# facebookresearch/seamless_communication

Hardware: AMD Instinct MI355X
Metric: S2ST utterances/sec (and real-time factor), seamlessM4T_v2_large, 10 s audio (higher is better)
Workload: dtype f32 activations x f16 weights, f32 accumulate

## Files before the change

include/seamless_hip_internal.h:

```cpp
#ifndef SEAMLESS_HIP_INTERNAL_H_
#define SEAMLESS_HIP_INTERNAL_H_

#include "seamless_hip.h"

#ifdef __cplusplus
extern "C" {
#endif

int sc_decoder_step_family(sc_model* m, int rows, int caller);

int sc_op_knob(const char* name, int dflt);

int sc_op_force_general_gemm(int on);
int32_t sc_op_voc_pack_plan(const int32_t* h_need, int32_t n, int64_t budget_rows, int32_t* h_group_first, int32_t cap);
int32_t sc_op_voc_tile_first(const int32_t* h_off, int32_t n, int32_t mul, int32_t tile_rows, int32_t* h_first);
int32_t sc_op_last_vocoder_packed_groups(sc_model* m);
int sc_op_single_plane(int on);
int sc_op_layernorm(const float* d_x, const float* d_gamma, const float* d_beta, float* d_y, int32_t rows, int32_t C,
                    int32_t act);
int sc_op_linear(const float* d_x, const void* d_w_f16, const float* d_bias, const float* d_res, float* d_y,
                 int32_t M, int32_t N, int32_t K, int32_t act, float alpha, int32_t split, int32_t force_gemv);
int sc_op_skinny_linear(const float* d_x, const void* d_w_f16, const float* d_bias, const float* d_res, float* d_y,
                        int32_t M, int32_t N, int32_t K, int32_t act, float alpha);
int sc_op_skinny_res_ln(const float* d_in, const void* d_w_f16, const float* d_bias, float* d_x_inout,
// ... 13 lines not shown
int sc_op_dstep_attention(const float* d_proj, int32_t S, const float* d_bias, float* d_kcache, float* d_vcache, int32_t cap,
                          int32_t pos, const int32_t* d_lens, int32_t cross, int32_t nb, int32_t heads, float* d_out);
int sc_op_dstep3_gemv(int32_t mode, const float* d_x, const void* d_w_f16, const float* d_bias, const float* d_gamma,
                      const float* d_beta, const float* d_res, float* d_y, float* d_h, int32_t M, int32_t N, int32_t K, int32_t act,
                      int32_t rg, int32_t shape);
int sc_op_dstep3_argmax(const float* d_x, const void* d_w_f16, int32_t M, int32_t N, int32_t K, int32_t step,
                        int32_t min_step_for_eos, int32_t force_eos_step, int32_t pad_idx, int32_t eos_idx, int32_t unk_idx,
                        float unk_penalty, int32_t* d_idx, float* d_lprob);
int sc_op_chain_bench(int32_t kind, int32_t rows, int32_t n, int32_t reps, float* us_per_kernel);
int sc_op_conv1d(const float* d_x, const void* d_w_f16_packed, const float* d_bias, const float* d_res, float* d_y,
                 int32_t nb, int32_t t_in, int32_t cin, int32_t cout, int32_t k, int32_t stride, int32_t pad,
                 int32_t dil, const int32_t* d_in_lens, int32_t in_act, int32_t act);
int sc_op_pack_conv_weight(const void* d_w_f16, void* d_dst_f16, int32_t cout, int32_t cin, int32_t k);
int sc_op_conv_transpose1d(const float* d_x, const void* d_v_f16, const void* d_g_f16, const float* d_bias,
                           float* d_y, int32_t nb, int32_t t_in, int32_t cin, int32_t cout, int32_t k,
                           int32_t stride, int32_t pad, int32_t in_act);
int sc_op_linear_presplit(const float* d_x, const void* d_w_f16, const float* d_bias, const float* d_res, float* d_y,
                          void* d_yh_f16, void* d_yl_f16, int32_t M, int32_t N, int32_t K, int32_t act, float alpha);
int sc_op_linear_presplit_argmax(const float* d_x, const void* d_w_f16, const float* d_bias, int32_t* d_idx, int32_t M, int32_t N,
                                 int32_t K);
int sc_op_conv1d_presplit(const float* d_x, const void* d_w_f16_packed, const float* d_bias, const float* d_res, float* d_y,
                          void* d_yh_f16, void* d_yl_f16, int32_t nb, int32_t t, int32_t cin, int32_t cout, int32_t k, int32_t pad,
                          int32_t dil, const unsigned char* d_row_valid, int32_t act);
int sc_op_resblock_pair_ps(const float* d_x, const void* d_w1_packed, const float* d_b1, const void* d_w2_packed, const float* d_b2,
                           float* d_out, int32_t nb, int32_t T, int32_t C, int32_t k, int32_t dil);
int sc_op_resblock_pair(const float* d_x, const void* d_w1_packed, const float* d_b1, const void* d_w2_packed,
                        const float* d_b2, float* d_out, int32_t nb, int32_t T, int32_t C, int32_t k, int32_t dil,
                        float slope, const float* d_avg_a, const float* d_avg_b);
int sc_op_mrf_fused(const float* d_x, const void* const* d_w1_packed, const float* const* d_b1, const void* const* d_w2_packed,
                    const float* const* d_b2, float* d_out, int32_t nb, int32_t T, int32_t C, const int32_t* k, const int32_t* dil,
                    float slope);
int sc_op_attention(const float* d_q, const float* d_k, const float* d_v, float* d_out, int32_t nb, int32_t heads,
                    int32_t sq, int32_t skv, int64_t ldq, int64_t ldk, int64_t ldv, int64_t ldo,
                    const int32_t* d_kv_lens, int32_t causal, const float* d_rel_k, int32_t rel_left,
                    int32_t rel_right);
int sc_op_attention_ex(const float* d_q, const float* d_k, const float* d_v, float* d_out, int32_t nb, int32_t heads,
                       int32_t sq, int32_t skv, int64_t ldq, int64_t ldk, int64_t ldv, int64_t ldo,
                       const int32_t* d_kv_lens, int32_t causal, const float* d_rel_k, int32_t rel_left,
                       int32_t rel_right, const int32_t* d_row_off, const float* d_rp_table, int64_t rp_ld,
                       const float* d_q_bias_u, const float* d_q_bias_v, void* d_out_hi, void* d_out_lo, int64_t ldoh);
int sc_op_glu_dwconv(const float* d_x, const float* d_w, float* d_y, int32_t nb, int32_t T, int32_t C, int32_t k,
                     const int32_t* d_lens);
int sc_op_glu_dwconv_ln(const float* d_x, const float* d_w, const float* d_gamma, const float* d_beta, int32_t act, void* d_yh_f16,
                        void* d_yl_f16, int32_t nb, int32_t T, int32_t C, int32_t k, const int32_t* d_lens, int32_t fused);
int sc_op_layernorm2(const float* d_x, const float* d_ga, const float* d_ba, const float* d_gb, const float* d_bb, float* d_y,
                     void* d_yh_f16, void* d_yl_f16, int32_t rows, int32_t C, int32_t fused);
// ... 67 lines not shown
```

seamless_communication_amd/_lib.py:

```python
from __future__ import annotations

import ctypes as C
from pathlib import Path
from typing import Optional

import os

_VARIANT = os.environ.get("SC_LIB_VARIANT", "")
LIB_PATH = Path(__file__).resolve().parent / (f"libseamless_hip.{_VARIANT}.so" if _VARIANT else "libseamless_hip.so")

SC_ABI_VERSION = 10
SC_MAX_UPSAMPLES = 8
SC_MAX_RESBLOCK_KERNELS = 4
SC_MAX_RESBLOCK_DILATIONS = 4
SC_F16, SC_F32, SC_I32 = 0, 1, 2


class SeamlessHipError(RuntimeError):
    pass


class sc_tensor_desc(C.Structure):
    _fields_ = [
        ("name", C.c_char_p),
# ... 147 lines not shown
    "sc_op_last_vocoder_packed_groups": (C.c_int32, [_P]),
    "sc_op_single_plane": (C.c_int, [C.c_int]),
    "sc_op_layernorm": (C.c_int, [_P, _P, _P, _P, _i, _i, _i]),
    "sc_op_linear": (C.c_int, [_P, _P, _P, _P, _P, _i, _i, _i, _i, C.c_float, _i, _i]),
    "sc_op_skinny_linear": (C.c_int, [_P, _P, _P, _P, _P, _i, _i, _i, _i, C.c_float]),
    "sc_op_skinny_res_ln": (C.c_int, [_P, _P, _P, _P, _P, _P, _P, _i, _i, _i, _i]),
    "sc_op_skinny_argmax": (C.c_int, [_P, _P, _i, _i, _i, _i, _i, _i, _i, _i, _i, C.c_float, _P, _P]),
    "sc_op_dstep_res_ln": (C.c_int, [_P, _P, _P, _P, _P, _P, _P, _i, _i, _i, _i]),
    "sc_op_dstep_linear_planes": (C.c_int, [_P, _P, _P, _P, _i, _i, _i, _i]),
    "sc_op_dstep_argmax": (C.c_int, [_P, _P, _i, _i, _i, _i, _i, _i, _i, _i, _i, C.c_float, _i, _P, _P]),
    "sc_op_resblock_pair_ps": (C.c_int, [_P, _P, _P, _P, _P, _P, _i, _i, _i, _i, _i]),
    "sc_op_glu_dwconv_ln": (C.c_int, [_P, _P, _P, _P, _i, _P, _P, _i, _i, _i, _i, _P, _i]),
    "sc_op_layernorm2": (C.c_int, [_P, _P, _P, _P, _P, _P, _P, _P, _i, _i, _i]),
    "sc_op_dstep3_gemv": (C.c_int, [_i, _P, _P, _P, _P, _P, _P, _P, _P, _i, _i, _i, _i, _i, _i]),
    "sc_op_dstep3_argmax": (C.c_int, [_P, _P, _i, _i, _i, _i, _i, _i, _i, _i, _i, C.c_float, _P, _P]),
    "sc_op_chain_bench": (C.c_int, [_i, _i, _i, _i, _P]),
    "sc_op_dstep_attention": (C.c_int, [_P, _i, _P, _P, _P, _i, _i, _P, _i, _i, _i, _P]),
    "sc_op_conv1d": (C.c_int, [_P, _P, _P, _P, _P, _i, _i, _i, _i, _i, _i, _i, _i, _P, _i, _i]),
    "sc_op_pack_conv_weight": (C.c_int, [_P, _P, _i, _i, _i]),
    "sc_op_conv_transpose1d": (C.c_int, [_P, _P, _P, _P, _P, _i, _i, _i, _i, _i, _i, _i, _i]),
    "sc_op_linear_presplit": (C.c_int, [_P, _P, _P, _P, _P, _P, _P, _i, _i, _i, _i, C.c_float]),
    "sc_op_linear_presplit_argmax": (C.c_int, [_P, _P, _P, _P, _i, _i, _i]),
    "sc_op_conv1d_presplit": (C.c_int, [_P, _P, _P, _P, _P, _P, _P, _i, _i, _i, _i, _i, _i, _i, _P, _i]),
    "sc_op_mrf_fused": (C.c_int, [_P, _P, _P, _P, _P, _P, _i, _i, _i, _P, _P, C.c_float]),
    "sc_op_resblock_pair": (C.c_int, [_P, _P, _P, _P, _P, _P, _i, _i, _i, _i, _i, C.c_float, _P, _P]),
    "sc_op_attention": (C.c_int, [_P, _P, _P, _P, _i, _i, _i, _i, C.c_int64, C.c_int64, C.c_int64, C.c_int64, _P, _i,
                                  _P, _i, _i]),
    "sc_op_attention_ex": (C.c_int, [_P, _P, _P, _P, _i, _i, _i, _i, C.c_int64, C.c_int64, C.c_int64, C.c_int64, _P, _i,
                                     _P, _i, _i, _P, _P, C.c_int64, _P, _P, _P, _P, C.c_int64]),
    "sc_op_glu_dwconv": (C.c_int, [_P, _P, _P, _i, _i, _i, _i, _P]),
    "sc_op_argmax": (C.c_int, [_P, _i, _i, _P, _P]),
    "sc_op_beam_candidates": (C.c_int, [_P, C.c_int64, _i, _i, _i, _P, _i, _i, _i, _i, _i, _i, C.c_float, _i, _P, _P, _P, _i, _i, _i,
                                        _P, _P, _i]),
    "sc_op_beam_candidates_banned": (C.c_int, [_P, C.c_int64, _i, _i, _i, _P, _i, _i, _i, _i, _i, _i, C.c_float, _i, _P, _P, _P, _i, _i,
                                               _i, _P, _P, _i, _P, _P, _i]),
    "sc_op_beam_select": (C.c_int, [_P, _P, _P, _P, _P, _P, _P, _P, _P, _P, _P, _P, _P, _P, _i, _P, _P, _i, _i, _i, _i, _i, _i, _i, _i,
                                    _i, C.c_float]),
    "sc_op_beam_compact": (C.c_int, [_P, _P, _P, _P, _P, _P, _P, _P, _P, _i, _i, _i, _i, _i, _i]),
    "sc_op_gather_cache": (C.c_int, [_P, _P, _P, _i, _i, _i, _i, _i, C.c_int64]),
    "sc_op_row_token_lprob": (C.c_int, [_P, C.c_int64, _i, _i, _i, _i, _P]),
    "sc_op_dstep_attention_ex": (C.c_int, [_P, _i, _P, _P, _P, _i, _i, _i, _P, _i, _i, _i, _P, _P, _P, _P, _i, _P, _P]),
    "sc_op_engine_step_close": (C.c_int, [_P, _P, _i, _i, _i, _i, _i, _i, _i, C.c_float, _P, _P, _i, _i, _P, _P, _P, _P, _P, _P, _P, _P]),
    "sc_op_engine_admit": (C.c_int, [_P, _i, _i, _i, _i, _P, _P, _P, _P, _P, _P, _P, _P, _P]),
    "sc_op_engine_set_slots": (C.c_int, [_P, _i, _i, _i, _P, _P, _P, _P]),
    "sc_op_engine_retire": (C.c_int, [_P, _P, _P, _i, _i, _i, _i, _P, _P, _P, _P, _P]),
    "sc_op_dstep3_embed_ex": (C.c_int, [_P, _P, C.c_float, _P, _i, _P, _P, _i, _i, _i, _i, _i, _P]),
# ... 96 lines not shown
```

seamless_communication_amd/csrc/api.hip:

```cpp
#include <atomic>
#include <cstring>
#include <map>
#include <mutex>
#include <set>

#include "../../include/seamless_hip_internal.h"
#include "engine.h"
#include "model.h"

using namespace sc;

struct sc_model {
    Model m;
};

struct sc_engine {
    std::unique_ptr<Engine> e;
    int device = 0;
    const void* weights = nullptr;
    std::set<sc_model*> attached;
};

static std::mutex g_attach_mu;
static std::map<Engine*, sc_engine*> g_engine_owner;
// ... 1200 lines not shown
    try {
        launch_split_f32(d_x, hi, lo, (int64_t)n, g_op_stream);
        Model tmp;
        Conv c;
        c.w = static_cast<const __half*>(d_w_f16_packed);
        c.b = d_bias;
        c.cout = cout;
        c.cin = cin;
        c.k = k;
        c.kpad = (int)align_up((int64_t)cin * k, 32);
        conv1d_presplit(tmp, hi, lo, c, d_res, d_y, static_cast<__half*>(d_yh_f16), static_cast<__half*>(d_yl_f16), nb, t, pad, dil,
                        d_row_valid, act);
        SC_HIP(hipStreamSynchronize(g_op_stream));
    } catch (...) {
        (void)hipFree(hi);
        (void)hipFree(lo);
        throw;
    }
    (void)hipFree(hi);
    (void)hipFree(lo);
    SC_API_END
}

int sc_op_resblock_pair_ps(const float* d_x, const void* d_w1_packed, const float* d_b1, const void* d_w2_packed, const float* d_b2,
                           float* d_out, int32_t nb, int32_t T, int32_t C, int32_t k, int32_t dil) {
    SC_API_BEGIN
    SC_CHECK(d_x && d_w1_packed && d_w2_packed && d_out && C % 32 == 0 && (k & 1), "sc_op_resblock_pair_ps: bad argument");
    OpScratch scratch;
    const size_t n = (size_t)nb * T * C;
    const bool one = g_op_single.load() != 0;
    __half* xh = scratch.get<__half>(n);
    __half* xl = one ? nullptr : scratch.get<__half>(n);
    __half* th = scratch.get<__half>(n);
    __half* tl = one ? nullptr : scratch.get<__half>(n);
    launch_lrelu_split_f32(d_x, 0.1f, xh, xl, (int64_t)n, g_op_stream);
    Model tmp;
    Conv c1, c2;
    c1.w = static_cast<const __half*>(d_w1_packed), c1.b = d_b1, c1.cin = c1.cout = C, c1.k = k, c1.kpad = C * k;
    c2.w = static_cast<const __half*>(d_w2_packed), c2.b = d_b2, c2.cin = c2.cout = C, c2.k = k, c2.kpad = C * k;
    conv1d_presplit(tmp, xh, xl, c1, nullptr, nullptr, th, tl, nb, T, (k * dil - dil) / 2, dil, nullptr, ACT_NONE, 0, nullptr, 0.1f, one ? 0 : 1);
    conv1d_presplit(tmp, th, tl, c2, d_x, d_out, nullptr, nullptr, nb, T, (k - 1) / 2, 1, nullptr, ACT_NONE, 0, nullptr, 0.1f, one ? 0 : 1);
    SC_HIP(hipStreamSynchronize(g_op_stream));
    SC_API_END
}

int sc_op_resblock_pair(const float* d_x, const void* d_w1_packed, const float* d_b1, const void* d_w2_packed,
// ... 576 lines not shown
```

seamless_communication_amd/csrc/common.cpp:

```cpp
#include "common.h"
#include <cstdlib>
#include <cstring>

namespace sc {

static thread_local char g_err[1024] = "";

void set_error(const char* fmt, ...) {
    va_list ap;
    va_start(ap, fmt);
    vsnprintf(g_err, sizeof(g_err), fmt, ap);
    va_end(ap);
}

const char* get_error() { return g_err; }

namespace knob {
namespace {
struct Knob {
    const char* name;
    int kind;
    const char* what;
};
const Knob knob_table[] = {
    {"SC_DEBUG_NUMERICS", 0, "honour the switches that change results"},
    {"SC_DEBUG_FILL", 0, "fill fresh scratch blocks with NaN (tests)"},
    {"SC_SPLIT_MODE", 1, "1: Conformer products on the hi fp16 plane only (precision study)"},
    {"SC_DECODER_GEN1", 1, "decoder step on the first-generation kernels"},
    {"SC_DECODER_GEN2", 1, "decoder step on the second-generation chain"},
    {"SC_DECODE_STEPWISE", 1, "teacher-forced pass step by step instead of one batched forward"},
    {"SC_VOC_SPLIT", 1, "vocoder ResBlock products on both fp16 planes of their activations again (bit 0 wide stages, bit 2 narrow stages); default: hi plane only"},
    {"SC_GEMM_GENERAL", 0, "general GEMM kernel instead of the fast path"}, {"SC_GEMM_PF2", 0, "GEMM prefetch depth"},
    {"SC_GEMM_GROUP_M", 0, "GEMM workgroup order"}, {"SC_GEMM_TILE", 0, "GEMM tile override"},
    {"SC_PS_TILE", 0, "DMA GEMM: largest tile"}, {"SC_PS_MIN256", 0, "DMA GEMM: tiles needed for 256 x 256"},
    {"SC_PS_MIN128", 0, "DMA GEMM: tiles needed for 128 x 128"},
    {"SC_PRESPLIT", 0, "0: Conformer operands split on the fly"}, {"SC_ENC_FUSE", 0, "0: separate Conformer element-wise launches"},
    {"SC_D3_RG_SMALL", 0, "decoder step: rows per row group, N = 1024 products"}, {"SC_D3_RG_FFN", 0, "decoder step: rows per row group, FFN-in"},
    {"SC_G3_STATIONARY", 0, "row-group products of wide steps: 0 one workgroup per row group, n = workgroup budget of the weight-stationary launch"},
    {"SC_G3_TILES", 0, "0: FFN-out of wide steps on the weight-stationary row-group walk instead of tile-owning waves"},
    {"SC_G3_TOUCH", 0, "weight-stationary products: bit 0 cooperative L2 touch of the activations, bit 1 K slices per XCD (FFN-out); default 3"},
    {"SC_D3_FFN_IN", 0, "decoder step: FFN-in workgroup shape"}, {"SC_D3_FFN_OUT", 0, "decoder step: FFN-out workgroup shape"},
    {"SC_T2U_GROUPS", 0, "NAR T2U: length buckets"}, {"SC_T2U_PACKED", 0, "0: NAR decoder on padded buckets"},
    {"SC_VOC_PS", 0, "0: vocoder wide stages on the register-staged convolution"}, {"SC_VOC_MRF", 0, "0: narrow vocoder stages as nine pair launches"},
    {"SC_VOC_GROUPS", 0, "vocoder: length buckets"}, {"SC_VOC_GROUP_OVERHEAD", 0, "vocoder: bucket planning overhead rows"},
    {"SC_VOC_STREAMS", 0, "vocoder: side chains"},
    {"SC_VOC_PACKED", 0, "0: ragged vocoder batches in length buckets on side chains instead of the packed pass"},
    {"SC_VOC_PACK_ROWS", 0, "vocoder: unit rows per packed group"},
    {"SC_ENGINE_RG_SMALL", 0, "decode engine: rows per row group, N = 1024 products"},
    {"SC_BEAM_COMPACT", 2, "0: beam search keeps finished utterances' slots"},
    {"SC_GREEDY_COMPACT", 2, "0: greedy generation keeps finished rows in their slots"}, {"SC_GREEDY_POLL", 2, "steps between looks at the finished flags"},
};
constexpr int N_KNOBS = sizeof(knob_table) / sizeof(knob_table[0]);
struct State {
    bool set[N_KNOBS];
    int val[N_KNOBS];
    bool numerics = false;
};
const State& state() {
// ... 58 lines not shown
```

seamless_communication_amd/csrc/k_gemm_ps.hip:

```cpp
#include <cstdlib>
#include <type_traits>

#include "kernels.h"

namespace sc {

typedef _Float16 half8_t __attribute__((ext_vector_type(8)));
typedef float float16_t __attribute__((ext_vector_type(16)));

namespace {

constexpr int PBK = 32;
#define SC_LDS_PTR(p) ((__attribute__((address_space(3))) void*)(p))

template <int ACT>
__device__ __forceinline__ float ps_act(float v) {
    if (ACT == ACT_RELU) return v > 0.f ? v : 0.f;
    if (ACT == ACT_SILU) return v / (1.f + expf(-v));
    if (ACT == ACT_TANH) return tanhf(v);
    return v;
}

typedef int i32x4_t __attribute__((ext_vector_type(4)));

// ... 52 lines not shown
                if (p.Cl)
                    *reinterpret_cast<h4_t*>(reinterpret_cast<_Float16*>(p.Cl) + m * p.ldcs + col) =
                        __builtin_convertvector(v - __builtin_convertvector(hi, f4_t), h4_t);
            }
        } else {
#pragma unroll
            for (int e = 0; e < 4; ++e) {
                if (col + e >= p.N) continue;
                float x = v[e];
                if (p.res && !dead) x += p.res[m * p.ldr + col + e];
                if (p.C) p.C[m * p.ldc + col + e] = x;
                if (p.Ch) {
                    if (p.plane_neg_slope != 1.0f) x = fmaxf(x, 0.f) + p.plane_neg_slope * fminf(x, 0.f);
                    const _Float16 h = (_Float16)x;
                    reinterpret_cast<_Float16*>(p.Ch)[m * p.ldcs + col + e] = h;
                    if (p.Cl) reinterpret_cast<_Float16*>(p.Cl)[m * p.ldcs + col + e] = (_Float16)(x - (float)h);
                }
            }
        }
    }
}

template <int BM, int BN, int WGM, int WGN, bool SPLIT, bool CONV, bool AMAX>
__global__ __launch_bounds__(WGM* WGN * 64) void gemm_ps_kernel(GemmPsArgs p, int tiles_n, int tiles_total, int tiles_per_xcd,
                                                                 uint32_t a_bytes, uint32_t w_bytes) {
    constexpr int NWAVE = WGM * WGN;
    constexpr bool ALTERNATE = SPLIT && NWAVE == 8;
    constexpr bool MID_BARRIER = SPLIT && !ALTERNATE;
    constexpr int WM = BM / WGM, WN = BN / WGN;
    constexpr int TM = WM / 32, TN = WN / 32;
    constexpr int ACH = BM / (16 * NWAVE);
    constexpr int BCH = BN / (16 * NWAVE);
    constexpr uint32_t OOB = 0x80000000u;
    constexpr int A_TILE = BM * 32, B_TILE = BN * 32;

    constexpr int A_PL = SPLIT ? 2 : 1;
    constexpr int STAGE_BYTES = (A_PL * A_TILE + B_TILE) * 2;
    constexpr int EPN = WN < 64 ? WN : (NWAVE * WM * (64 + 4) * 4 <= 3 * STAGE_BYTES ? 64 : 32);
    constexpr int EP_LD = EPN + 4;
    static_assert(NWAVE * WM * EP_LD * 4 <= 3 * STAGE_BYTES, "epilogue tiles must fit in the stage memory");
    __shared__ __attribute__((aligned(16))) char smem[3 * STAGE_BYTES];
    _Float16* const sAh0 = reinterpret_cast<_Float16*>(smem);
    _Float16* const sAl0 = sAh0 + (A_PL - 1) * A_TILE;
    _Float16* const sB0 = sAh0 + A_PL * A_TILE;
    _Float16* const sAh1 = reinterpret_cast<_Float16*>(smem + STAGE_BYTES);
    _Float16* const sAl1 = sAh1 + (A_PL - 1) * A_TILE;
    _Float16* const sB1 = sAh1 + A_PL * A_TILE;
    _Float16* const sAh2 = reinterpret_cast<_Float16*>(smem + 2 * STAGE_BYTES);
    _Float16* const sAl2 = sAh2 + (A_PL - 1) * A_TILE;
    _Float16* const sB2 = sAh2 + A_PL * A_TILE;

    const int bid = blockIdx.x;
    const int tile = (bid & 7) * tiles_per_xcd + (bid >> 3);
    if (tile >= tiles_total) return;
    const int tm = tile / tiles_n;
    const int tn = tile - tm * tiles_n;
    const int tid = threadIdx.x, lane = tid & 63, wave = tid >> 6;
    const int wm = wave / WGN, wn = wave % WGN;
    const int m0 = tm * BM, n0 = tn * BN;

    const i32x4_t rah = make_rsrc_words(p.Ah, a_bytes);
    const i32x4_t ral = make_rsrc_words(p.Al, a_bytes);
    const i32x4_t rw = make_rsrc_words(p.W, w_bytes);

    uint32_t a_voff[ACH], b_voff[BCH];
    int a_t[ACH];
    int a_len[ACH];
#pragma unroll
    for (int j = 0; j < ACH; ++j) {
        const int row = 16 * (wave * ACH + j) + (lane >> 2);
        const int seg = (lane & 3) ^ ((row >> 2) & 3);
        a_voff[j] = (m0 + row) < p.M ? (uint32_t)(((int64_t)(m0 + row) * p.lda + seg * 8) * 2) : OOB;
        a_t[j] = 0;
        a_len[j] = 0;
        if (CONV) {
            if (p.row_pos) {
                const int2 rp = (m0 + row) < p.M ? p.row_pos[m0 + row] : make_int2(0, 0);
                a_t[j] = rp.x;
                a_len[j] = rp.y;
            } else {
                a_t[j] = (m0 + row) % p.rows_per_item;
                a_len[j] = p.rows_per_item;
            }
        }
    }
    int nx_tap = 0, nx_cs = 0, nx_slab = 0;
    const int spt = CONV ? p.conv_cin / PBK : 1;
    const uint32_t row_bytes = (uint32_t)(p.lda * 2);
    uint32_t va_[ACH];
    int ka_ = 0;
#define PS_NEXT_ADDR()                                                                                  \
    do {                                                                                                \
        if (CONV) {                                                                                     \
            const int dt_ = nx_tap * p.conv_dil - p.conv_pad;                                           \
            ka_ = nx_cs * (PBK * 2);                                                                    \
            _Pragma("unroll") for (int j = 0; j < ACH; ++j) {                                           \
                const bool in_ = (uint32_t)(a_t[j] + dt_) < (uint32_t)a_len[j] && a_voff[j] != OOB;     \
                va_[j] = in_ ? a_voff[j] + (uint32_t)dt_ * row_bytes : OOB;                             \
            }                                                                                           \
            if (++nx_cs == spt) {                                                                       \
                nx_cs = 0;                                                                              \
                ++nx_tap;                                                                               \
            }                                                                                           \
        } else {                                                                                        \
            ka_ = nx_slab * (PBK * 2);                                                                  \
            _Pragma("unroll") for (int j = 0; j < ACH; ++j) va_[j] = a_voff[j];                         \
        }                                                                                               \
        ++nx_slab;                                                                                      \
    } while (0)
#pragma unroll
    for (int j = 0; j < BCH; ++j) {
        const int row = 16 * (wave * BCH + j) + (lane >> 2);
        const int seg = (lane & 3) ^ ((row >> 2) & 3);
        b_voff[j] = (n0 + row) < p.N ? (uint32_t)(((int64_t)(n0 + row) * p.ldw + seg * 8) * 2) : OOB;
    }

    float16_t acc[TM][TN];
#pragma unroll
    for (int i = 0; i < TM; ++i)
#pragma unroll
        for (int j = 0; j < TN; ++j)
#pragma unroll
            for (int r = 0; r < 16; ++r) acc[i][j][r] = 0.f;

    int a_off[TM][2], b_off[TN][2];
#pragma unroll
    for (int kc = 0; kc < 2; ++kc) {
        const int s = kc * 2 + (lane >> 5);
#pragma unroll
        for (int i = 0; i < TM; ++i) a_off[i][kc] = swz(wm * WM + i * 32 + (lane & 31), s);
#pragma unroll
        for (int j = 0; j < TN; ++j) b_off[j][kc] = swz(wn * WN + j * 32 + (lane & 31), s);
    }

#define PS_DMA(RSRC, LDSP, VOFF, SOFF)                                                                        \
    asm volatile("s_mov_b32 m0, %0\n\tbuffer_load_dwordx4 %1, %2, %3 offen lds"                              \
                 :                                                                                            \
                 : "s"(__builtin_amdgcn_readfirstlane((int)(uint32_t)(uintptr_t)SC_LDS_PTR(LDSP))), "v"(VOFF), \
                   "s"(RSRC), "s"((int)(SOFF))                                                                \
                 : "memory")
#define PS_ISSUE(AH, AL, BB, KOFF)                                                             \
    do {                                                                                       \
        PS_NEXT_ADDR();                                                                        \
        _Pragma("unroll") for (int j = 0; j < ACH; ++j) {                                      \
            PS_DMA(rah, &AH[(wave * ACH + j) * 512], va_[j], ka_);                             \
            if (SPLIT) PS_DMA(ral, &AL[(wave * ACH + j) * 512], va_[j], ka_);                  \
        }                                                                                      \
        _Pragma("unroll") for (int j = 0; j < BCH; ++j)                                        \
            PS_DMA(rw, &BB[(wave * BCH + j) * 512], b_voff[j], (KOFF));                        \
    } while (0)

    constexpr int NDMA = 2 * ACH + BCH;
    constexpr int NLIVE = SPLIT ? NDMA : ACH + BCH;
    static_assert(NDMA == 6 || NDMA == 3, "two or one 1 KB chunk per operand and wave");
    static_assert(NLIVE < 16, "vmcnt(NLIVE) in the low bits of s_waitcnt");

// ... 22 lines not shown
        }                                                                                                              \
        if (more_) PS_NEXT_ADDR();                                                                                     \
        __builtin_amdgcn_sched_barrier(0);                                                                             \
        int q_ = 0;                                                                                                    \
        _Pragma("unroll") for (int kc = 0; kc < 2; ++kc) {                                                             \
            _Pragma("unroll") for (int i = 0; i < TM; ++i)                                                             \
                _Pragma("unroll") for (int j = 0; j < TN; ++j) {                                                       \
                    acc[i][j] = __builtin_amdgcn_mfma_f32_32x32x16_f16(ah[kc][i], bf[kc][j], acc[i][j], 0, 0, 0);       \
                    if (q_ < NDMA) {                                                                                   \
                        __builtin_amdgcn_sched_barrier(0);                                                             \
                        if (more_) PS_DMA_Q(q_, NAH, NAH, NB, ((S) + 2) * (PBK * 2));                                  \
                        __builtin_amdgcn_sched_barrier(0);                                                             \
                    }                                                                                                  \
                    ++q_;                                                                                              \
                }                                                                                                      \
        }                                                                                                              \
                 \
        _Pragma("unroll") for (int q2 = 2 * TM * TN; q2 < NDMA; ++q2)                                                  \
            if (more_) PS_DMA_Q(q2, NAH, NAH, NB, ((S) + 2) * (PBK * 2));                                              \
        asm volatile("" ::: "memory");                                                                                 \
    } while (0)

    const int nslab = p.K / PBK;
    if constexpr (ALTERNATE) {
        static_assert(NDMA == 6, "the alternating schedule is written for the split 8-wave tile");
        constexpr int NH = NDMA / 2;
        const bool grp_b = __builtin_amdgcn_readfirstlane(wave) >= NWAVE / 2;
        half8_t f_ah[TM], f_al[TM], f_bf[TN];
#define PP_LOADSEG(S, KC, CAH, CAL, CB, NAH, NAL, NB)                                           \
    do {                                                                                        \
        _Pragma("unroll") for (int j = 0; j < TN; ++j) f_bf[j] = PS_LDS8(CB, b_off[j][KC]);     \
        _Pragma("unroll") for (int i = 0; i < TM; ++i) {                                        \
            f_ah[i] = PS_LDS8(CAH, a_off[i][KC]);                                               \
            f_al[i] = PS_LDS8(CAL, a_off[i][KC]);                                               \
        }                                                                                       \
        __builtin_amdgcn_sched_barrier(0);                                                      \
        if ((S) + 2 < nslab) {                                                                  \
            if ((KC) == 0) PS_NEXT_ADDR();                                                      \
            _Pragma("unroll") for (int q = (KC) * NH; q < (KC) * NH + NH; ++q) PS_DMA_Q(q, NAH, NAL, NB, ((S) + 2) * (PBK * 2)); \
        }                                                                                       \
        __builtin_amdgcn_s_waitcnt(0xC07F);                    \
        __builtin_amdgcn_sched_barrier(0);                                                      \
    } while (0)
#define PP_COMPUTE()                                                                                               \
    do {                                                                                                           \
        __builtin_amdgcn_s_setprio(1);                                                                             \
// ... 16 lines not shown
        else if ((S) > 0) PP_COMPUTE();                                                         \
        PP_BARRIER();                                                                           \
        if (!(ROLE_B)) PP_COMPUTE();                                                            \
        else PP_LOADSEG(S, 0, CAH, CAL, CB, NAH, NAL, NB);                                      \
        PP_BARRIER();                                                                           \
        if (!(ROLE_B)) PP_LOADSEG(S, 1, CAH, CAL, CB, NAH, NAL, NB);                            \
        else PP_COMPUTE();                                                                      \
        PP_BARRIER();                                                                           \
        if (!(ROLE_B)) PP_COMPUTE();                                                            \
        else PP_LOADSEG(S, 1, CAH, CAL, CB, NAH, NAL, NB);                                      \
        if ((S) + 2 < nslab) __builtin_amdgcn_s_waitcnt(0x0076);       \
        else __builtin_amdgcn_s_waitcnt(0x0070);                                                \
        PP_BARRIER();                                                                           \
    } while (0)
#define PP_LOOP(ROLE_B)                                                                         \
    do {                                                                                        \
        for (int s = 0; s < nslab; s += 3) {                                                    \
            PP_STEP(ROLE_B, s, sAh0, sAl0, sB0, sAh2, sAl2, sB2);                               \
            if (s + 1 < nslab) PP_STEP(ROLE_B, s + 1, sAh1, sAl1, sB1, sAh0, sAl0, sB0);        \
            if (s + 2 < nslab) PP_STEP(ROLE_B, s + 2, sAh2, sAl2, sB2, sAh1, sAl1, sB1);        \
        }                                                                                       \
        if (ROLE_B) PP_COMPUTE();                              \
    } while (0)
        PS_ISSUE(sAh0, sAl0, sB0, 0);
        if (nslab > 1) PS_ISSUE(sAh1, sAl1, sB1, PBK * 2);
        if (nslab > 1) __builtin_amdgcn_s_waitcnt(0x0076);
        else __builtin_amdgcn_s_waitcnt(0x0070);
        PP_BARRIER();
        if (grp_b) PP_LOOP(true);
        else PP_LOOP(false);
#undef PP_LOOP
#undef PP_STEP
#undef PP_BARRIER
#undef PP_LOADSEG
#undef PP_COMPUTE
    } else if constexpr (MID_BARRIER) {
        constexpr int NH = NDMA / 2;
        half8_t c_ah[TM], c_al[TM], c_bf[TN];
#define PS_READ_C0(AH, AL, BB)                                                                  \
    do {                                                                                        \
        _Pragma("unroll") for (int i = 0; i < TM; ++i) {                                        \
            c_ah[i] = PS_LDS8(AH, a_off[i][0]);                                                 \
            c_al[i] = PS_LDS8(AL, a_off[i][0]);                                                 \
        }                                                                                       \
        _Pragma("unroll") for (int j = 0; j < TN; ++j) c_bf[j] = PS_LDS8(BB, b_off[j][0]);      \
    } while (0)
#define PS_HSTEP(S, CAH, CAL, CB, NAH, NAL, NB, OAH, OAL, OB)                                                          \
    do {                                                                                                               \
// ... 24 lines not shown
            else __builtin_amdgcn_s_waitcnt(0x0070);                                          \
            __builtin_amdgcn_s_barrier();                                                                              \
            asm volatile("" ::: "memory");                                                                             \
            PS_READ_C0(NAH, NAL, NB);                                                                                  \
        }                                                                                                              \
        const bool iss3_ = (S) + 3 < nslab;                                                                            \
        if (iss3_) PS_NEXT_ADDR();                                                                                     \
        __builtin_amdgcn_sched_barrier(0);                                                                             \
        q_ = 0;                                                                                                        \
        _Pragma("unroll") for (int i = 0; i < TM; ++i)                                                                 \
            _Pragma("unroll") for (int j = 0; j < TN; ++j) {                                                           \
                acc[i][j] = __builtin_amdgcn_mfma_f32_32x32x16_f16(ah1[i], bf1[j], acc[i][j], 0, 0, 0);                 \
                acc[i][j] = __builtin_amdgcn_mfma_f32_32x32x16_f16(al1[i], bf1[j], acc[i][j], 0, 0, 0);                 \
                if (q_ < NH) {                                                                                         \
                    __builtin_amdgcn_sched_barrier(0);                                                                 \
                    if (iss3_) PS_DMA_Q(q_, CAH, CAL, CB, ((S) + 3) * (PBK * 2));                                      \
                    __builtin_amdgcn_sched_barrier(0);                                                                 \
                }                                                                                                      \
                ++q_;                                                                                                  \
            }                                                                                                          \
        asm volatile("" ::: "memory");                                                                                 \
    } while (0)

        PS_ISSUE(sAh0, sAl0, sB0, 0);
        if (nslab > 1) PS_ISSUE(sAh1, sAl1, sB1, PBK * 2);
        if (nslab > 2) {
            PS_NEXT_ADDR();
#pragma unroll
            for (int q = 0; q < NH; ++q) PS_DMA_Q(q, sAh2, sAl2, sB2, 2 * (PBK * 2));
        }
        if (nslab > 2) __builtin_amdgcn_s_waitcnt(NDMA == 6 ? 0x0079 : 0x0074);
        else if (nslab > 1) __builtin_amdgcn_s_waitcnt(NDMA == 6 ? 0x0076 : 0x0073);
        else __builtin_amdgcn_s_waitcnt(0x0070);
        __builtin_amdgcn_s_barrier();
        asm volatile("" ::: "memory");
        PS_READ_C0(sAh0, sAl0, sB0);
        for (int s = 0; s < nslab; s += 3) {
            PS_HSTEP(s, sAh0, sAl0, sB0, sAh1, sAl1, sB1, sAh2, sAl2, sB2);
            if (s + 1 < nslab) PS_HSTEP(s + 1, sAh1, sAl1, sB1, sAh2, sAl2, sB2, sAh0, sAl0, sB0);
            if (s + 2 < nslab) PS_HSTEP(s + 2, sAh2, sAl2, sB2, sAh0, sAl0, sB0, sAh1, sAl1, sB1);
        }
#undef PS_HSTEP
#undef PS_READ_C0
    } else {
        PS_ISSUE(sAh0, sAl0, sB0, 0);
        if (nslab > 1) PS_ISSUE(sAh1, sAl1, sB1, PBK * 2);
        for (int s = 0; s < nslab; s += 3) {
            PS_STEP(s, sAh0, sB0, sAh2, sB2);
            if (s + 1 < nslab) PS_STEP(s + 1, sAh1, sB1, sAh0, sB0);
            if (s + 2 < nslab) PS_STEP(s + 2, sAh2, sB2, sAh1, sB1);
        }
    }
#undef PS_STEP
#undef PS_LDS8
#undef PS_DMA_Q
#undef PS_NEXT_ADDR
#undef PS_ISSUE
#undef PS_DMA

    __builtin_amdgcn_s_waitcnt(0x0070);
    __builtin_amdgcn_s_barrier();
    asm volatile("" ::: "memory");
    float* ep = reinterpret_cast<float*>(smem) + wave * (WM * EP_LD);
    const int m0w = m0 + wm * WM;
    float am_best = -INFINITY;
    int am_idx = 0x7fffffff;
    auto pass = [&](auto hc) {
        constexpr int h = decltype(hc)::value;
#pragma unroll
        for (int i = 0; i < TM; ++i)
#pragma unroll
            for (int j = 0; j < EPN / 32; ++j)
#pragma unroll
                for (int r = 0; r < 16; ++r)
                    ep[(i * 32 + (r & 3) + 8 * (r >> 2) + 4 * (lane >> 5)) * EP_LD + j * 32 + (lane & 31)] = acc[i][h * (EPN / 32) + j][r];
        const int n0w = n0 + wn * WN + h * EPN;
        if constexpr (AMAX) {
            typedef float f4_t __attribute__((ext_vector_type(4)));
            if (lane < WM) {
                const float* row = ep + lane * EP_LD;
#pragma unroll
                for (int c4 = 0; c4 < EPN / 4; ++c4) {
                    const f4_t a = *reinterpret_cast<const f4_t*>(row + 4 * c4);
#pragma unroll
                    for (int e = 0; e < 4; ++e) {
                        const int col = n0w + 4 * c4 + e;
                        if (col < p.N) {
                            const float v = (a[e] + (p.bias ? p.bias[col] : 0.f)) * p.alpha;
                            if (v > am_best) {
                                am_best = v;
                                am_idx = col;
                            }
                        }
                    }
                }
            }
            return;
        }
        if (p.act == ACT_NONE) ps_epilogue<WM, EPN, EP_LD, ACT_NONE>(p, ep, m0w, n0w, lane);
        else if (p.act == ACT_RELU) ps_epilogue<WM, EPN, EP_LD, ACT_RELU>(p, ep, m0w, n0w, lane);
        else if (p.act == ACT_SILU) ps_epilogue<WM, EPN, EP_LD, ACT_SILU>(p, ep, m0w, n0w, lane);
        else ps_epilogue<WM, EPN, EP_LD, ACT_TANH>(p, ep, m0w, n0w, lane);
    };
    static_assert(WN % EPN == 0 && WN / EPN >= 1 && WN / EPN <= 4, "one to four epilogue passes");
    pass(std::integral_constant<int, 0>{});
    if constexpr (WN / EPN > 1) pass(std::integral_constant<int, 1>{});
    if constexpr (WN / EPN > 2) pass(std::integral_constant<int, 2>{});
    if constexpr (WN / EPN > 3) pass(std::integral_constant<int, 3>{});
    if constexpr (AMAX) {
        const int64_t m = m0w + lane;
        if (lane < WM && m < p.M) p.amax[m * p.amax_ld + tn * WGN + wn] = make_float2(am_best, __int_as_float(am_idx));
    }
}

template <int BM, int BN, int WGM, int WGN>
void launch_ps_cfg(const GemmPsArgs& a, hipStream_t s) {
    const int tiles_m = cdiv(a.M, BM), tiles_n = cdiv(a.N, BN);
    const int tiles_total = tiles_m * tiles_n;
    const int tiles_per_xcd = cdiv(tiles_total, 8);
    char name[64];
    snprintf(name, sizeof(name), "gemm_%dx%d_presplit", BM, BN);
    prof::Scope scope(name, 2.0 * a.M * (double)a.N * a.K,
                      4.0 * a.M * (double)a.K + 2.0 * a.N * (double)a.K + (a.amax ? 8.0 * a.M * (double)a.amax_ld : 4.0 * a.M * (double)a.N * (a.res ? 2.0 : 1.0)), s);
    const dim3 grid(tiles_per_xcd * 8), block(WGM * WGN * 64);
    const uint32_t ab = (uint32_t)((int64_t)a.M * a.lda * 2), wb = (uint32_t)((int64_t)a.N * a.ldw * 2);
    const auto launch = [&](auto kernel) { hipLaunchKernelGGL(kernel, grid, block, 0, s, a, tiles_n, tiles_total, tiles_per_xcd, ab, wb); };
    const bool conv = a.conv_taps > 0;
    if (a.amax) launch(gemm_ps_kernel<BM, BN, WGM, WGN, true, false, true>);
    else if (a.split && conv) launch(gemm_ps_kernel<BM, BN, WGM, WGN, true, true, false>);
    else if (a.split) launch(gemm_ps_kernel<BM, BN, WGM, WGN, true, false, false>);
    else if (conv) launch(gemm_ps_kernel<BM, BN, WGM, WGN, false, true, false>);
    else launch(gemm_ps_kernel<BM, BN, WGM, WGN, false, false, false>);
}

int ps_tile(int M, int N) {
    static const int max_tile = knob::value("SC_PS_TILE", 256);
    const int64_t tiles128 = (int64_t)cdiv(M, 128) * cdiv(N, 128);
    const int64_t tiles256 = (int64_t)cdiv(M, 256) * cdiv(N, 256);
    static const int min256 = knob::value("SC_PS_MIN256", 224);
    static const int min128 = knob::value("SC_PS_MIN128", 256);
    if (max_tile >= 256 && tiles256 >= min256 && N > 128) return 256;
    return tiles128 >= min128 ? 128 : 64;
}

}

void launch_gemm_presplit(const GemmPsArgs& a, hipStream_t s) {
    SC_CHECK(a.Ah && (a.Al || !a.split) && a.W && (a.C || a.Ch || a.amax), "presplit gemm: null operand");
    SC_CHECK(a.Ch || !a.Cl, "presplit gemm: a lo output plane needs its hi plane");
// ... 68 lines not shown
```

Baseline: 334.4.

## Add persistent-workgroup mode to 256x256 DMA GEMM with next-tile prefetch under epilogue

The 8-wave presplit GEMM kernel can now run as persistent workgroups that walk tiles within their XCD slice. While one tile's epilogue runs, the kernel issues the next tile's first DMA stage, using a separate LDS region for the epilogue scratch so the two do not collide. Persistence is enabled by the SC_PS_PERSIST knob, which defaults to 0. With the default, the grid is unchanged, but the 8-wave kernel still uses a larger LDS footprint and a fixed EPN of 32, which may reduce occupancy. A packed-item conv1d presplit API entry is also added.

```diff
diff --git a/include/seamless_hip_internal.h b/include/seamless_hip_internal.h
--- a/include/seamless_hip_internal.h
+++ b/include/seamless_hip_internal.h
@@ -59,6 +59,9 @@
 int sc_op_conv1d_presplit(const float* d_x, const void* d_w_f16_packed, const float* d_bias, const float* d_res, float* d_y,
                           void* d_yh_f16, void* d_yl_f16, int32_t nb, int32_t t, int32_t cin, int32_t cout, int32_t k, int32_t pad,
                           int32_t dil, const unsigned char* d_row_valid, int32_t act);
+int sc_op_conv1d_presplit_packed(const float* d_x, const void* d_w_f16_packed, const float* d_bias, const float* d_res, float* d_y,
+                                 void* d_yh_f16, void* d_yl_f16, const int32_t* d_item_off, int32_t n_items, int32_t rows, int32_t cin,
+                                 int32_t cout, int32_t k, int32_t pad, int32_t dil, int32_t act, int32_t split);
 int sc_op_resblock_pair_ps(const float* d_x, const void* d_w1_packed, const float* d_b1, const void* d_w2_packed, const float* d_b2,
                            float* d_out, int32_t nb, int32_t T, int32_t C, int32_t k, int32_t dil);
 int sc_op_resblock_pair(const float* d_x, const void* d_w1_packed, const float* d_b1, const void* d_w2_packed,
diff --git a/seamless_communication_amd/_lib.py b/seamless_communication_amd/_lib.py
--- a/seamless_communication_amd/_lib.py
+++ b/seamless_communication_amd/_lib.py
@@ -193,6 +193,7 @@
     "sc_op_linear_presplit": (C.c_int, [_P, _P, _P, _P, _P, _P, _P, _i, _i, _i, _i, C.c_float]),
     "sc_op_linear_presplit_argmax": (C.c_int, [_P, _P, _P, _P, _i, _i, _i]),
     "sc_op_conv1d_presplit": (C.c_int, [_P, _P, _P, _P, _P, _P, _P, _i, _i, _i, _i, _i, _i, _i, _P, _i]),
+    "sc_op_conv1d_presplit_packed": (C.c_int, [_P, _P, _P, _P, _P, _P, _P, _P, _i, _i, _i, _i, _i, _i, _i, _i, _i]),
     "sc_op_mrf_fused": (C.c_int, [_P, _P, _P, _P, _P, _P, _i, _i, _i, _P, _P, C.c_float]),
     "sc_op_resblock_pair": (C.c_int, [_P, _P, _P, _P, _P, _P, _i, _i, _i, _i, _i, C.c_float, _P, _P]),
     "sc_op_attention": (C.c_int, [_P, _P, _P, _P, _i, _i, _i, _i, C.c_int64, C.c_int64, C.c_int64, C.c_int64, _P, _i,
diff --git a/seamless_communication_amd/csrc/api.hip b/seamless_communication_amd/csrc/api.hip
--- a/seamless_communication_amd/csrc/api.hip
+++ b/seamless_communication_amd/csrc/api.hip
@@ -1246,6 +1246,28 @@
     SC_API_END
 }
 
+int sc_op_conv1d_presplit_packed(const float* d_x, const void* d_w_f16_packed, const float* d_bias, const float* d_res, float* d_y,
+                                 void* d_yh_f16, void* d_yl_f16, const int32_t* d_item_off, int32_t n_items, int32_t rows, int32_t cin,
+                                 int32_t cout, int32_t k, int32_t pad, int32_t dil, int32_t act, int32_t split) {
+    SC_API_BEGIN
+    SC_CHECK(d_x && d_w_f16_packed && (d_y || d_yh_f16) && d_item_off && n_items > 0 && rows > 0, "sc_op_conv1d_presplit_packed: null argument");
+    SC_CHECK(split || !d_yl_f16, "sc_op_conv1d_presplit_packed: split = 0 produces no lo plane");
+    OpScratch scratch;
+    const size_t n = (size_t)rows * cin;
+    __half* hi = scratch.get<__half>(n);
+    __half* lo = split ? scratch.get<__half>(n) : nullptr;
+    int2* row_pos = scratch.get<int2>((size_t)rows);
+    launch_lrelu_split_f32(d_x, 1.0f, hi, lo, (int64_t)n, g_op_stream);
+    launch_item_row_pos(d_item_off, n_items, 1, rows, row_pos, g_op_stream);
+    Model tmp;
+    Conv c;
+    c.w = static_cast<const __half*>(d_w_f16_packed), c.b = d_bias, c.cout = cout, c.cin = cin, c.k = k, c.kpad = cin * k;
+    conv1d_presplit(tmp, hi, lo, c, d_res, d_y, static_cast<__half*>(d_yh_f16), static_cast<__half*>(d_yl_f16), 0, 0, pad, dil, nullptr, act,
+                    rows, row_pos, 1.0f, split ? 1 : 0);
+    SC_HIP(hipStreamSynchronize(g_op_stream));
+    SC_API_END
+}
+
 int sc_op_resblock_pair_ps(const float* d_x, const void* d_w1_packed, const float* d_b1, const void* d_w2_packed, const float* d_b2,
                            float* d_out, int32_t nb, int32_t T, int32_t C, int32_t k, int32_t dil) {
     SC_API_BEGIN
diff --git a/seamless_communication_amd/csrc/common.cpp b/seamless_communication_amd/csrc/common.cpp
--- a/seamless_communication_amd/csrc/common.cpp
+++ b/seamless_communication_amd/csrc/common.cpp
@@ -34,6 +34,8 @@
     {"SC_GEMM_GROUP_M", 0, "GEMM workgroup order"}, {"SC_GEMM_TILE", 0, "GEMM tile override"},
     {"SC_PS_TILE", 0, "DMA GEMM: largest tile"}, {"SC_PS_MIN256", 0, "DMA GEMM: tiles needed for 256 x 256"},
     {"SC_PS_MIN128", 0, "DMA GEMM: tiles needed for 128 x 128"},
+    {"SC_PS_PERSIST", 0, "1: 256 x 256 DMA GEMM as persistent workgroups (tile walk, hand-over under the epilogue)"},
+    {"SC_PS_WGS", 0, "256 x 256 DMA GEMM: persistent workgroups (0: one per CU)"},
     {"SC_PRESPLIT", 0, "0: Conformer operands split on the fly"}, {"SC_ENC_FUSE", 0, "0: separate Conformer element-wise launches"},
     {"SC_D3_RG_SMALL", 0, "decoder step: rows per row group, N = 1024 products"}, {"SC_D3_RG_FFN", 0, "decoder step: rows per row group, FFN-in"},
     {"SC_G3_STATIONARY", 0, "row-group products of wide steps: 0 one workgroup per row group, n = workgroup budget of the weight-stationary launch"},
diff --git a/seamless_communication_amd/csrc/k_gemm_ps.hip b/seamless_communication_amd/csrc/k_gemm_ps.hip
--- a/seamless_communication_amd/csrc/k_gemm_ps.hip
+++ b/seamless_communication_amd/csrc/k_gemm_ps.hip
@@ -1,3 +1,4 @@
+#include <algorithm>
 #include <cstdlib>
 #include <type_traits>
 
@@ -98,9 +99,10 @@
 }
 
 template <int BM, int BN, int WGM, int WGN, bool SPLIT, bool CONV, bool AMAX>
-__global__ __launch_bounds__(WGM* WGN * 64) void gemm_ps_kernel(GemmPsArgs p, int tiles_n, int tiles_total, int tiles_per_xcd,
+__global__ __launch_bounds__(WGM* WGN * 64) void gemm_ps_kernel(GemmPsArgs p, int tiles_n, int tiles_total, int tiles_per_xcd, int tile_step,
                                                                  uint32_t a_bytes, uint32_t w_bytes) {
     constexpr int NWAVE = WGM * WGN;
+    constexpr bool PERSIST = NWAVE == 8;
     constexpr bool ALTERNATE = SPLIT && NWAVE == 8;
     constexpr bool MID_BARRIER = SPLIT && !ALTERNATE;
     constexpr int WM = BM / WGM, WN = BN / WGN;
@@ -112,10 +114,14 @@
 
     constexpr int A_PL = SPLIT ? 2 : 1;
     constexpr int STAGE_BYTES = (A_PL * A_TILE + B_TILE) * 2;
-    constexpr int EPN = WN < 64 ? WN : (NWAVE * WM * (64 + 4) * 4 <= 3 * STAGE_BYTES ? 64 : 32);
+    constexpr int EPN = PERSIST ? 32 : WN < 64 ? WN : (NWAVE * WM * (64 + 4) * 4 <= 3 * STAGE_BYTES ? 64 : 32);
     constexpr int EP_LD = EPN + 4;
-    static_assert(NWAVE * WM * EP_LD * 4 <= 3 * STAGE_BYTES, "epilogue tiles must fit in the stage memory");
-    __shared__ __attribute__((aligned(16))) char smem[3 * STAGE_BYTES];
+    constexpr int EP_BASE = PERSIST ? STAGE_BYTES : 0;
+    constexpr int EP_END = EP_BASE + NWAVE * WM * EP_LD * 4;
+    constexpr int SMEM_BYTES = EP_END > 3 * STAGE_BYTES ? EP_END : 3 * STAGE_BYTES;
+    static_assert(PERSIST || EP_END <= 3 * STAGE_BYTES, "epilogue tiles must fit in the stage memory");
+    static_assert(SMEM_BYTES <= 160 * 1024 && EP_BASE % 16 == 0, "LDS of a CU");
+    __shared__ __attribute__((aligned(16))) char smem[SMEM_BYTES];
     _Float16* const sAh0 = reinterpret_cast<_Float16*>(smem);
     _Float16* const sAl0 = sAh0 + (A_PL - 1) * A_TILE;
     _Float16* const sB0 = sAh0 + A_PL * A_TILE;
@@ -127,13 +133,13 @@
     _Float16* const sB2 = sAh2 + A_PL * A_TILE;
 
     const int bid = blockIdx.x;
-    const int tile = (bid & 7) * tiles_per_xcd + (bid >> 3);
-    if (tile >= tiles_total) return;
-    const int tm = tile / tiles_n;
-    const int tn = tile - tm * tiles_n;
-    const int tid = threadIdx.x, lane = tid & 63, wave = tid >> 6;
+    const int tile_end = min(((bid & 7) + 1) * tiles_per_xcd, tiles_total);
+    int tile = (bid & 7) * tiles_per_xcd + (bid >> 3);
+    if (tile >= tile_end) return;
+    const int tid = threadIdx.x, lane = tid & 63;
+    const int wave = PERSIST ? __builtin_amdgcn_readfirstlane(tid >> 6) : tid >> 6;
     const int wm = wave / WGN, wn = wave % WGN;
-    const int m0 = tm * BM, n0 = tn * BN;
+    int tn, m0, n0;
 
     const i32x4_t rah = make_rsrc_words(p.Ah, a_bytes);
     const i32x4_t ral = make_rsrc_words(p.Al, a_bytes);
@@ -142,25 +148,37 @@
     uint32_t a_voff[ACH], b_voff[BCH];
     int a_t[ACH];
     int a_len[ACH];
-#pragma unroll
-    for (int j = 0; j < ACH; ++j) {
-        const int row = 16 * (wave * ACH + j) + (lane >> 2);
-        const int seg = (lane & 3) ^ ((row >> 2) & 3);
-        a_voff[j] = (m0 + row) < p.M ? (uint32_t)(((int64_t)(m0 + row) * p.lda + seg * 8) * 2) : OOB;
-        a_t[j] = 0;
-        a_len[j] = 0;
-        if (CONV) {
-            if (p.row_pos) {
-                const int2 rp = (m0 + row) < p.M ? p.row_pos[m0 + row] : make_int2(0, 0);
-                a_t[j] = rp.x;
-                a_len[j] = rp.y;
-            } else {
-                a_t[j] = (m0 + row) % p.rows_per_item;
-                a_len[j] = p.rows_per_item;
-            }
-        }
-    }
     int nx_tap = 0, nx_cs = 0, nx_slab = 0;
+#define PS_SETUP_TILE(T)                                                                                             \
+    do {                                                                                                             \
+        const int tm_ = (T) / tiles_n;                                                                               \
+        tn = (T) - tm_ * tiles_n;                                                                                    \
+        m0 = tm_ * BM;                                                                                               \
+        n0 = tn * BN;                                                                                                \
+        _Pragma("unroll") for (int j = 0; j < ACH; ++j) {                                                            \
+            const int row = 16 * (wave * ACH + j) + (lane >> 2);                                                     \
+            const int seg = (lane & 3) ^ ((row >> 2) & 3);                                                           \
+            a_voff[j] = (m0 + row) < p.M ? (uint32_t)(((int64_t)(m0 + row) * p.lda + seg * 8) * 2) : OOB;            \
+            a_t[j] = 0;                                                                                              \
+            a_len[j] = 0;                                                                                            \
+            if (CONV) {                                                                                              \
+                if (p.row_pos) {                                                                                     \
+                    const int2 rp = (m0 + row) < p.M ? p.row_pos[m0 + row] : make_int2(0, 0);                        \
+                    a_t[j] = rp.x;                                                                                   \
+                    a_len[j] = rp.y;                                                                                 \
+                } else {                                                                                             \
+                    a_t[j] = (m0 + row) % p.rows_per_item;                                                           \
+                    a_len[j] = p.rows_per_item;                                                                      \
+                }                                                                                                    \
+            }                                                                                                        \
+        }                                                                                                            \
+        _Pragma("unroll") for (int j = 0; j < BCH; ++j) {                                                            \
+            const int row = 16 * (wave * BCH + j) + (lane >> 2);                                                     \
+            const int seg = (lane & 3) ^ ((row >> 2) & 3);                                                           \
+            b_voff[j] = (n0 + row) < p.N ? (uint32_t)(((int64_t)(n0 + row) * p.ldw + seg * 8) * 2) : OOB;            \
+        }                                                                                                            \
+        nx_tap = 0, nx_cs = 0, nx_slab = 0;                                                                          \
+    } while (0)
     const int spt = CONV ? p.conv_cin / PBK : 1;
     const uint32_t row_bytes = (uint32_t)(p.lda * 2);
     uint32_t va_[ACH];
@@ -184,30 +202,20 @@
         }                                                                                               \
         ++nx_slab;                                                                                      \
     } while (0)
-#pragma unroll
-    for (int j = 0; j < BCH; ++j) {
-        const int row = 16 * (wave * BCH + j) + (lane >> 2);
-        const int seg = (lane & 3) ^ ((row >> 2) & 3);
-        b_voff[j] = (n0 + row) < p.N ? (uint32_t)(((int64_t)(n0 + row) * p.ldw + seg * 8) * 2) : OOB;
-    }
 
     float16_t acc[TM][TN];
-#pragma unroll
-    for (int i = 0; i < TM; ++i)
-#pragma unroll
-        for (int j = 0; j < TN; ++j)
-#pragma unroll
-            for (int r = 0; r < 16; ++r) acc[i][j][r] = 0.f;
 
     int a_off[TM][2], b_off[TN][2];
-#pragma unroll
-    for (int kc = 0; kc < 2; ++kc) {
-        const int s = kc * 2 + (lane >> 5);
-#pragma unroll
-        for (int i = 0; i < TM; ++i) a_off[i][kc] = swz(wm * WM + i * 32 + (lane & 31), s);
-#pragma unroll
-        for (int j = 0; j < TN; ++j) b_off[j][kc] = swz(wn * WN + j * 32 + (lane & 31), s);
-    }
+#define PS_FRAG_OFFSETS()                                                                                            \
+    do {                                                                                                             \
+        int l_ = lane;                                                                                               \
+        if (PERSIST) asm volatile("" : "+v"(l_));                                                                    \
+        _Pragma("unroll") for (int kc = 0; kc < 2; ++kc) {                                                           \
+            const int s = kc * 2 + (l_ >> 5);                                                                        \
+            _Pragma("unroll") for (int i = 0; i < TM; ++i) a_off[i][kc] = swz(wm * WM + i * 32 + (l_ & 31), s);      \
+            _Pragma("unroll") for (int j = 0; j < TN; ++j) b_off[j][kc] = swz(wn * WN + j * 32 + (l_ & 31), s);      \
+        }                                                                                                            \
+    } while (0)
 
 #define PS_DMA(RSRC, LDSP, VOFF, SOFF)                                                                        \
     asm volatile("s_mov_b32 m0, %0\n\tbuffer_load_dwordx4 %1, %2, %3 offen lds"                              \
@@ -276,6 +284,17 @@
     } while (0)
 
     const int nslab = p.K / PBK;
+    PS_SETUP_TILE(tile);
+    PS_ISSUE(sAh0, sAl0, sB0, 0);
+    if (nslab > 1) PS_ISSUE(sAh1, sAl1, sB1, PBK * 2);
+  for (;;) {
+    PS_FRAG_OFFSETS();
+#pragma unroll
+    for (int i = 0; i < TM; ++i)
+#pragma unroll
+        for (int j = 0; j < TN; ++j)
+#pragma unroll
+            for (int r = 0; r < 16; ++r) acc[i][j][r] = 0.f;
     if constexpr (ALTERNATE) {
         static_assert(NDMA == 6, "the alternating schedule is written for the split 8-wave tile");
         constexpr int NH = NDMA / 2;
@@ -338,8 +357,6 @@
         }                                                                                       \
         if (ROLE_B) PP_COMPUTE();                              \
     } while (0)
-        PS_ISSUE(sAh0, sAl0, sB0, 0);
-        if (nslab > 1) PS_ISSUE(sAh1, sAl1, sB1, PBK * 2);
         if (nslab > 1) __builtin_amdgcn_s_waitcnt(0x0076);
         else __builtin_amdgcn_s_waitcnt(0x0070);
         PP_BARRIER();
@@ -410,8 +427,6 @@
         asm volatile("" ::: "memory");                                                                                 \
     } while (0)
 
-        PS_ISSUE(sAh0, sAl0, sB0, 0);
-        if (nslab > 1) PS_ISSUE(sAh1, sAl1, sB1, PBK * 2);
         if (nslab > 2) {
             PS_NEXT_ADDR();
 #pragma unroll
@@ -431,26 +446,33 @@
 #undef PS_HSTEP
 #undef PS_READ_C0
     } else {
-        PS_ISSUE(sAh0, sAl0, sB0, 0);
-        if (nslab > 1) PS_ISSUE(sAh1, sAl1, sB1, PBK * 2);
         for (int s = 0; s < nslab; s += 3) {
             PS_STEP(s, sAh0, sB0, sAh2, sB2);
             if (s + 1 < nslab) PS_STEP(s + 1, sAh1, sB1, sAh0, sB0);
             if (s + 2 < nslab) PS_STEP(s + 2, sAh2, sB2, sAh1, sB1);
         }
     }
-#undef PS_STEP
-#undef PS_LDS8
-#undef PS_DMA_Q
-#undef PS_NEXT_ADDR
-#undef PS_ISSUE
-#undef PS_DMA
 
     __builtin_amdgcn_s_waitcnt(0x0070);
     __builtin_amdgcn_s_barrier();
     asm volatile("" ::: "memory");
-    float* ep = reinterpret_cast<float*>(smem) + wave * (WM * EP_LD);
-    const int m0w = m0 + wm * WM;
+    const int e_tn = tn, e_m0 = m0, e_n0 = n0;
+    int next = 0;
+    bool more = false;
+    if constexpr (PERSIST) {
+        next = tile + tile_step;
+        more = next < tile_end;
+        if (more) {
+            PS_SETUP_TILE(next);
+            PS_ISSUE(sAh0, sAl0, sB0, 0);
+        }
+    }
+    int lane_e_ = lane;
+    if constexpr (PERSIST) asm volatile("" : "+v"(lane_e_));
+    {
+    const int lane = lane_e_;
+    float* ep = reinterpret_cast<float*>(smem + EP_BASE) + wave * (WM * EP_LD);
+    const int m0w = e_m0 + wm * WM;
     float am_best = -INFINITY;
     int am_idx = 0x7fffffff;
     auto pass = [&](auto hc) {
@@ -462,7 +484,7 @@
 #pragma unroll
                 for (int r = 0; r < 16; ++r)
                     ep[(i * 32 + (r & 3) + 8 * (r >> 2) + 4 * (lane >> 5)) * EP_LD + j * 32 + (lane & 31)] = acc[i][h * (EPN / 32) + j][r];
-        const int n0w = n0 + wn * WN + h * EPN;
+        const int n0w = e_n0 + wn * WN + h * EPN;
         if constexpr (AMAX) {
             typedef float f4_t __attribute__((ext_vector_type(4)));
             if (lane < WM) {
@@ -497,8 +519,33 @@
     if constexpr (WN / EPN > 3) pass(std::integral_constant<int, 3>{});
     if constexpr (AMAX) {
         const int64_t m = m0w + lane;
-        if (lane < WM && m < p.M) p.amax[m * p.amax_ld + tn * WGN + wn] = make_float2(am_best, __int_as_float(am_idx));
-    }
+        if (lane < WM && m < p.M) p.amax[m * p.amax_ld + e_tn * WGN + wn] = make_float2(am_best, __int_as_float(am_idx));
+    }
+    }
+    if (!more) break;
+    __builtin_amdgcn_s_waitcnt(0xC07F);
+    __builtin_amdgcn_s_barrier();
+    asm volatile("" ::: "memory");
+    if (nslab > 1) PS_ISSUE(sAh1, sAl1, sB1, PBK * 2);
+    tile = next;
+  }
+#undef PS_STEP
+#undef PS_LDS8
+#undef PS_DMA_Q
+#undef PS_NEXT_ADDR
+#undef PS_ISSUE
+#undef PS_SETUP_TILE
+#undef PS_FRAG_OFFSETS
+#undef PS_DMA
+}
+
+int persistent_wgs() {
+    static const int n = [] {
+        int dev = 0, cus = 0;
+        if (hipGetDevice(&dev) != hipSuccess || hipDeviceGetAttribute(&cus, hipDeviceAttributeMultiprocessorCount, dev) != hipSuccess) cus = 0;
+        return cus >= 8 ? cus / 8 * 8 : 8;
+    }();
+    return n;
 }
 
 template <int BM, int BN, int WGM, int WGN>
@@ -506,13 +553,20 @@
     const int tiles_m = cdiv(a.M, BM), tiles_n = cdiv(a.N, BN);
     const int tiles_total = tiles_m * tiles_n;
     const int tiles_per_xcd = cdiv(tiles_total, 8);
+    int wgs = tiles_per_xcd * 8;
+    if (WGM * WGN == 8) {
+        static const int persist = knob::value("SC_PS_PERSIST", 0);
+        static const int wgs_knob = knob::value("SC_PS_WGS", 0);
+        if (persist) wgs = wgs_knob > 0 ? (int)align_up((int64_t)wgs_knob, 8) : std::min(wgs, persistent_wgs());
+    }
+    const int tile_step = wgs / 8;
     char name[64];
     snprintf(name, sizeof(name), "gemm_%dx%d_presplit", BM, BN);
     prof::Scope scope(name, 2.0 * a.M * (double)a.N * a.K,
                       4.0 * a.M * (double)a.K + 2.0 * a.N * (double)a.K + (a.amax ? 8.0 * a.M * (double)a.amax_ld : 4.0 * a.M * (double)a.N * (a.res ? 2.0 : 1.0)), s);
-    const dim3 grid(tiles_per_xcd * 8), block(WGM * WGN * 64);
+    const dim3 grid(wgs), block(WGM * WGN * 64);
     const uint32_t ab = (uint32_t)((int64_t)a.M * a.lda * 2), wb = (uint32_t)((int64_t)a.N * a.ldw * 2);
-    const auto launch = [&](auto kernel) { hipLaunchKernelGGL(kernel, grid, block, 0, s, a, tiles_n, tiles_total, tiles_per_xcd, ab, wb); };
+    const auto launch = [&](auto kernel) { hipLaunchKernelGGL(kernel, grid, block, 0, s, a, tiles_n, tiles_total, tiles_per_xcd, tile_step, ab, wb); };
     const bool conv = a.conv_taps > 0;
     if (a.amax) launch(gemm_ps_kernel<BM, BN, WGM, WGN, true, false, true>);
     else if (a.split && conv) launch(gemm_ps_kernel<BM, BN, WGM, WGN, true, true, false>);
```

Result: slower. 328.6 (-1.7%).
